# matthewdm0816/BridgeQA

Measured on AMD Instinct MI355X. Metric: train samples/s (40k-pt scene + 512^2 view, bs16), higher is better.
Workload: dtype bf16

## Files before the change

### bridgeqa_amd/csrc/gemm_mid.hip

```cpp
#include "gemm_common.h"

#ifndef BQ_MID_ABLATE
#define BQ_MID_ABLATE 0
#endif

namespace bq {

typedef __attribute__((address_space(3))) unsigned char lds_u8_t;
typedef unsigned u32x2_t __attribute__((ext_vector_type(2)));
typedef unsigned u32x4_t __attribute__((ext_vector_type(4)));

template <bool P_XC, bool Q_XC, int EPI, bool OUT_F32, int ST_AUX, bool SK = false>
__global__ __launch_bounds__(256, 2) void gemm128_kernel(const GemmArgs args) {
  static_assert(!OUT_F32 || (P_XC && Q_XC && EPI == EPI_NONE), "fp32 out = the weight-gradient form");
  static_assert(!Q_XC || OUT_F32, "a contraction-major Q = the weight-gradient form");
  static_assert(!SK || (!OUT_F32 && EPI != EPI_BIAS_GELU), "stream-K: bf16 out, one output");
  __shared__ __attribute__((aligned(16))) unsigned char smem[65536 + 4 * 2048 + (SK ? 16 : 0)];
  const int tid = threadIdx.x;
  const int lane = tid & 63;
  const int wave = __builtin_amdgcn_readfirstlane(tid >> 6);
  const int wr = wave >> 1, wc = wave & 1;
  const int nwg = args.total_tiles, G = (int)gridDim.x;

  const int row16 = lane & 15, q4 = lane >> 4, cp = lane & 7, lr = lane >> 3;
  const int kc_base = row16 * 128 + ((q4 ^ (row16 & 7)) << 4);
  const int xc_q = (lane & 15) >> 2;
  const int xcg = (xc_q >> 1) | ((q4 & 1) << 1), xc0 = (8 * q4 + xc_q) * 128 + 8 * (lane & 3);
  constexpr int PA0 = 0, PA1 = 16384, QB = 32768;
  const int uA0 = PA0 + wr * 8192, uA1 = PA1 + wr * 8192;
  const int bsub = wc * 2;

  struct Tile { int pi, i0, j0, nkt, kt0, t; };
  auto xcd_order = [](int v, int n) {
    const int q = n >> 3, r = n & 7, x = v & 7;
    return (x < r ? x * (q + 1) : r * (q + 1) + (x - r) * q) + (v >> 3);
  };
  auto decode_t = [&](int t) {
    int pi = 0;
    for (int k = 1; k < args.n; ++k)
      if (t >= args.p[k].tile0) pi = k;
    const GemmProblem &pr = args.p[pi];
    const int tl = t - pr.tile0;
    const int tiles_j = (pr.Nj + 127) >> 7;
    Tile tt;
    tt.pi = pi;
    tt.j0 = (tiles_j - 1 - tl / pr.tiles_i()) * 128;
    tt.i0 = (tl % pr.tiles_i()) * 256;
    tt.nkt = (pr.Kc + 63) >> 6;
    tt.kt0 = 0;
    tt.t = t;
    return tt;
  };
  auto decode = [&](int v) { return decode_t(xcd_order(v, nwg)); };
  const int nkt_full = SK ? (args.p[0].Kc + 63) >> 6 : 1;
  const int U = SK ? nwg * nkt_full : 0;
  auto bound = [&](int x) {
    int b = (int)((long)x * U / G);
    const int r = b % nkt_full;
    return r == 1 ? b - 1 : (r == nkt_full - 1 ? b + 1 : b);
  };
  auto seg = [&](int u, int ue) {
    const int t = u / nkt_full;
    Tile tt = decode_t(t);
    tt.kt0 = u - t * nkt_full;
    const int left = nkt_full - tt.kt0;
    tt.nkt = left < ue - u ? left : ue - u;
    return tt;
  };
  const int slot = SK ? xcd_order((int)blockIdx.x, G) : 0;
  int su = SK ? bound(slot) : 0;
  const int sue = SK ? bound(slot + 1) : 0;

  unsigned vP[2], vQ[2];
  unsigned stepP[2], dgP[2], ddP[2], ddQ[2], stepQ[2];
  int remP[2], remQ[2];
  int rsrcP_pi[2], rsrcQ_pi[2];
  const unsigned DEAD = 0x80000000u;
  const int ur0 = wave * 8 + lr;

  auto set_p = [&](int half, const Tile &tt, bool live) {
    const GemmProblem &pr = args.p[tt.pi];
    const int ldp = pr.ldp;
    unsigned v;
    if (!P_XC) v = (unsigned)(((tt.i0 + half * 64 + ur0) * ldp + (cp ^ (ur0 & 7)) * 8) * 2);
    else v = (unsigned)((ur0 * ldp + tt.i0 + half * 64 + (cp ^ (xg(ur0) << 1)) * 8) * 2);
    stepP[half] = P_XC ? (unsigned)(64 * ldp * 2) : 128u;
    if (SK) v += (unsigned)tt.kt0 * stepP[half];
    vP[half] = live ? v : DEAD;
    dgP[half] = P_XC ? 256u : (unsigned)(128 * ldp * 2);
    ddP[half] = (unsigned)(32 * ldp * 2);
    remP[half] = live ? tt.nkt : 0x40000000;
    rsrcP_pi[half] = tt.pi;
  };
  auto set_q = [&](int half, const Tile &tt, bool live) {
    const GemmProblem &pr = args.p[tt.pi];
    unsigned v;
    if (!Q_XC) {
      const int row0 = tt.j0 + half * 32 + ur0;
      const unsigned o0 = mapped_row(row0, pr.ldq, pr.q_rpb(), pr.q_bstride);
      v = (o0 + (unsigned)((cp ^ (ur0 & 7)) * 8)) * 2u;
      ddQ[half] = pr.q_rpb() ? (mapped_row(row0 + 64, pr.ldq, pr.q_rpb(), pr.q_bstride) - o0) * 2u : (unsigned)(64 * pr.ldq * 2);
    } else {
      const int c = cp ^ (xg(ur0) << 1);
      v = (unsigned)((ur0 * pr.ldq + tt.j0 + (c >> 2) * 64 + half * 32 + (c & 3) * 8) * 2);
      ddQ[half] = (unsigned)(32 * pr.ldq * 2);
    }
    stepQ[half] = Q_XC ? (unsigned)(64 * pr.ldq * 2) : 128u;
    if (SK) v += (unsigned)tt.kt0 * stepQ[half];
    vQ[half] = live ? v : DEAD;
    remQ[half] = live ? tt.nkt : 0x40000000;
    rsrcQ_pi[half] = tt.pi;
  };

  int v = blockIdx.x;
  Tile cur = SK ? seg(su, sue) : decode(v);
  bool has_next = SK ? (su + cur.nkt < sue) : (v + G < nwg);
  Tile nxt = has_next ? (SK ? seg(su + cur.nkt, sue) : decode(v + G)) : cur;

  auto dma_p = [&](int half) {
    const GemmProblem &pr = args.p[rsrcP_pi[half]];
    const auto rs = __builtin_amdgcn_make_buffer_rsrc((void *)pr.P, 0, pr.p_bytes, 0x00020000);
#pragma unroll
    for (int g = 0; g < 2; ++g)
#pragma unroll
      for (int d = 0; d < 2; ++d)
        if (BQ_MID_ABLATE != 2)
          __builtin_amdgcn_raw_ptr_buffer_load_lds(rs, (lds_void_t *)(smem + (half ? PA1 : PA0) + g * 8192 + (wave + 4 * d) * 1024),
                                                   16, vP[half] + (g * dgP[half] + d * ddP[half]), 0, 0, 0);
    vP[half] += stepP[half];
    if (--remP[half] == 0) set_p(half, nxt, has_next);
  };
  auto dma_q = [&](int half, unsigned par) {
    const GemmProblem &pr = args.p[rsrcQ_pi[half]];
    const auto rs = __builtin_amdgcn_make_buffer_rsrc((void *)pr.Q, 0, pr.q_bytes, 0x00020000);
#pragma unroll
    for (int d = 0; d < 2; ++d)
      if (BQ_MID_ABLATE != 2)
        __builtin_amdgcn_raw_ptr_buffer_load_lds(rs, (lds_void_t *)(smem + QB + (par & 1) * 16384 + half * 8192 + (wave + 4 * d) * 1024),
                                                 16, vQ[half] + d * ddQ[half], 0, 0, 0);
    vQ[half] += Q_XC ? stepQ[half] : 128u;
    if (--remQ[half] == 0) set_q(half, nxt, has_next);
  };

  set_q(0, cur, true); set_q(1, cur, true); set_p(0, cur, true); set_p(1, cur, true);
  unsigned gk = 0;
  dma_q(0, 0); dma_q(1, 0); dma_p(0); dma_q(0, 1); dma_p(1);

  f32x4 acc[8][4];
  bf16x8 fa[4][2], fb0[2][2], fb1[2][2];
#define BQ_MID_MFMA(AO, FB, BO)                                                                       \
  _Pragma("unroll") for (int kk = 0; kk < 2; ++kk) _Pragma("unroll") for (int a = 0; a < 4; ++a)      \
      _Pragma("unroll") for (int b = 0; b < 2; ++b) if (BQ_MID_ABLATE != 1 || (a == 0 && b == 0)) acc[AO + a][BO + b] =  \
          __builtin_amdgcn_mfma_f32_16x16x32_bf16(fa[a][kk], FB[b][kk], acc[AO + a][BO + b], 0, 0, 0);
#define BQ_MID_COMPUTE_BEGIN()                              \
  asm volatile("s_waitcnt lgkmcnt(0)" ::: "memory");        \
  __builtin_amdgcn_sched_barrier(0);                        \
  __builtin_amdgcn_s_setprio(1);
#define BQ_MID_COMPUTE_END()                                \
  __builtin_amdgcn_s_setprio(0);                            \
  __builtin_amdgcn_sched_barrier(0);
  constexpr int NPASS = (EPI == EPI_BIAS_GELU) ? 2 : 1;
  constexpr int NSTORE = OUT_F32 ? 36 : 16 * NPASS;
  bf16x8 ones;
  f32x4 qs[4];
  if (OUT_F32) {
#pragma unroll
    for (int e = 0; e < 8; ++e) ones[e] = (__bf16)1.0f;
  }
#define BQ_MID_QSUM(FB, BO)                                                                           \
  if (OUT_F32 && do_qsum) {                                                                           \
    _Pragma("unroll") for (int kk = 0; kk < 2; ++kk) _Pragma("unroll") for (int b = 0; b < 2; ++b)    \
        qs[BO + b] = __builtin_amdgcn_mfma_f32_16x16x32_bf16(ones, FB[b][kk], qs[BO + b], 0, 0, 0);   \
  }

  for (bool first = true;; first = false) {
    const GemmProblem &pr = args.p[cur.pi];
    const int Ni = pr.Ni, Nj = pr.Nj;
    const int iw = cur.i0 + wr * 128, jw = cur.j0 + wc * 64;
    const bool vA0 = iw < Ni, vA1 = iw + 64 < Ni, vB0 = jw < Nj, vB1 = jw + 32 < Nj;
#pragma unroll
    for (int a = 0; a < 8; ++a)
#pragma unroll
      for (int b = 0; b < 4; ++b) acc[a][b] = f32x4{0.f, 0.f, 0.f, 0.f};
    const bool do_qsum = OUT_F32 && pr.colsum != nullptr && cur.i0 == 0 && wr == 0;
    if (OUT_F32) {
#pragma unroll
      for (int b = 0; b < 4; ++b) qs[b] = f32x4{0.f, 0.f, 0.f, 0.f};
    }

    for (int kt = 0; kt < cur.nkt; ++kt, ++gk) {
      const unsigned char *qb = smem + QB + (gk & 1) * 16384;
      const bool after_stores = kt == 0 && !first;
      const bool last = kt == cur.nkt - 1;
      if (after_stores) wait_vmcnt<6 + NSTORE>(); else wait_vmcnt<6>();
      BQ_BARRIER();
#pragma unroll
      for (int a = 0; a < 4; ++a)
#pragma unroll
        for (int kk = 0; kk < 2; ++kk) fa[a][kk] = read_frag_cf_x<P_XC>(smem + uA0, a, kk, kc_base, xc0, xcg);
#pragma unroll
      for (int b = 0; b < 2; ++b)
#pragma unroll
        for (int kk = 0; kk < 2; ++kk) fb0[b][kk] = read_frag_cf_x<Q_XC>(qb, bsub + b, kk, kc_base, xc0, xcg);
      dma_q(1, gk + 1);
      BQ_MID_COMPUTE_BEGIN();
      if (vA0 && vB0) { BQ_MID_MFMA(0, fb0, 0) }
      if (vB0) { BQ_MID_QSUM(fb0, 0) }
      BQ_MID_COMPUTE_END();
      BQ_BARRIER();
#pragma unroll
      for (int b = 0; b < 2; ++b)
#pragma unroll
        for (int kk = 0; kk < 2; ++kk) fb1[b][kk] = read_frag_cf_x<Q_XC>(qb + 8192, bsub + b, kk, kc_base, xc0, xcg);
      dma_p(0);
      BQ_MID_COMPUTE_BEGIN();
      if (vA0 && vB1) { BQ_MID_MFMA(0, fb1, 2) }
      if (vB1) { BQ_MID_QSUM(fb1, 2) }
      BQ_MID_COMPUTE_END();
      if (after_stores) wait_vmcnt<6 + NSTORE>(); else wait_vmcnt<6>();
      BQ_BARRIER();
#pragma unroll
      for (int a = 0; a < 4; ++a)
#pragma unroll
        for (int kk = 0; kk < 2; ++kk) fa[a][kk] = read_frag_cf_x<P_XC>(smem + uA1, a, kk, kc_base, xc0, xcg);
      if (!last) dma_q(0, gk + 2);
      BQ_MID_COMPUTE_BEGIN();
      if (vA1 && vB1) { BQ_MID_MFMA(4, fb1, 2) }
      BQ_MID_COMPUTE_END();
      BQ_BARRIER();
      if (!last) dma_p(1);
      __builtin_amdgcn_sched_barrier(0);
      __builtin_amdgcn_s_setprio(1);
      if (vA1 && vB0) { BQ_MID_MFMA(4, fb0, 0) }
      BQ_MID_COMPUTE_END();
    }

    bool sk_partial = false;
    if (SK && cur.nkt != nkt_full) {
      unsigned *tick = (unsigned *)args.sk_ws + 2 * cur.t;
      float *slabs = (float *)((char *)args.sk_ws + SK_TICKET_BYTES);
      const int t0 = cur.t * nkt_full, t1 = t0 + nkt_full;
      int s_lo = slot, s_hi = slot;
      while (s_lo > 0 && bound(s_lo) > t0) --s_lo;
      while (s_hi + 1 < G && bound(s_hi + 1) < t1) ++s_hi;
      const int n_part = s_hi - s_lo + 1;
      const unsigned flag_lds = (unsigned)(size_t)((lds_u8_t *)smem) + 65536u + 4u * 2048u;
      if (wave == 0) {
        unsigned old = 0;
        if (lane == 0) old = __hip_atomic_fetch_add(tick, 1u, __ATOMIC_RELAXED, __HIP_MEMORY_SCOPE_AGENT);
        old = (unsigned)__builtin_amdgcn_readfirstlane((int)old);
        asm volatile("ds_write_b32 %0, %1\n\ts_waitcnt lgkmcnt(0)" ::"v"(flag_lds), "v"(old) : "memory");
      }
      BQ_BARRIER();
      unsigned arrived;
      asm volatile("ds_read_b32 %0, %1\n\ts_waitcnt lgkmcnt(0)" : "=v"(arrived) : "v"(flag_lds) : "memory");
      arrived = (unsigned)__builtin_amdgcn_readfirstlane((int)arrived);
      const auto rsW = __builtin_amdgcn_make_buffer_rsrc((void *)slabs, 0, (unsigned)(2 * G) * (unsigned)SK_SLAB_BYTES > 0x7fffffffu
                                                         ? 0x7fffffffu : (unsigned)(2 * G) * (unsigned)SK_SLAB_BYTES, 0x00020000);
      auto slab_off = [&](int sl) { return (unsigned)((2 * sl + (bound(sl) >= t0 ? 0 : 1))) * (unsigned)SK_SLAB_BYTES; };
      if (arrived != (unsigned)(n_part - 1)) {
        sk_partial = true;
        __builtin_amdgcn_sched_barrier(0);
        dma_q(0, gk + 1);
        dma_p(1);
        __builtin_amdgcn_sched_barrier(0);
        const unsigned base = slab_off(slot) + (unsigned)(wave * 32 * 1024 + lane * 16);
#pragma unroll
        for (int a = 0; a < 8; ++a)
#pragma unroll
          for (int b = 0; b < 4; ++b)
            __builtin_amdgcn_raw_buffer_store_b128(__builtin_bit_cast(u32x4_t, acc[a][b]), rsW, base + (unsigned)((a * 4 + b) * 1024), 0, 16);
        asm volatile("s_waitcnt vmcnt(0)" ::: "memory");
        BQ_BARRIER();
        if (wave == 0 && lane == 0) __hip_atomic_fetch_add(tick + 1, 1u, __ATOMIC_RELAXED, __HIP_MEMORY_SCOPE_AGENT);
      } else {
        if (wave == 0 && lane == 0) {
          for (int spin = 0; spin < (1 << 22) && __hip_atomic_load(tick + 1, __ATOMIC_RELAXED, __HIP_MEMORY_SCOPE_AGENT) != (unsigned)(n_part - 1); ++spin)
            __builtin_amdgcn_s_sleep(4);
          __hip_atomic_store(tick, 0u, __ATOMIC_RELAXED, __HIP_MEMORY_SCOPE_AGENT);
          __hip_atomic_store(tick + 1, 0u, __ATOMIC_RELAXED, __HIP_MEMORY_SCOPE_AGENT);
        }
        BQ_BARRIER();
        for (int sl = s_lo; sl <= s_hi; ++sl) {
          if (sl == slot) continue;
          const unsigned base = slab_off(sl) + (unsigned)(wave * 32 * 1024 + lane * 16);
#pragma unroll
          for (int a0 = 0; a0 < 8; a0 += 4) {
            u32x4_t part[16];
#pragma unroll
            for (int e = 0; e < 16; ++e)
              part[e] = __builtin_amdgcn_raw_buffer_load_b128(rsW, base + (unsigned)((a0 * 4 + e) * 1024), 0, 16);
            asm volatile("s_waitcnt vmcnt(0)" ::: "memory");
            __builtin_amdgcn_sched_barrier(0);
#pragma unroll
            for (int e = 0; e < 16; ++e) acc[a0 + (e >> 2)][e & 3] += __builtin_bit_cast(f32x4, part[e]);
          }
        }
      }
    }

    if (SK && sk_partial) {
    } else if (OUT_F32) {
      __builtin_amdgcn_sched_barrier(0);
      dma_q(0, gk + 1);
      dma_p(1);
      __builtin_amdgcn_sched_barrier(0);
      const int ldo = pr.ldo;
      const auto rsO = __builtin_amdgcn_make_buffer_rsrc(pr.out, 0, (unsigned)((long)Nj * ldo * 4), 0x00020000);
      const auto rsS = __builtin_amdgcn_make_buffer_rsrc((void *)pr.colsum, 0, pr.colsum == nullptr ? 0u : (unsigned)(Nj * 4), 0x00020000);
#pragma unroll
      for (int b = 0; b < 4; ++b) {
        const int j = jw + b * 16 + row16;
        __builtin_amdgcn_raw_buffer_store_b32(__float_as_uint(qs[b][0]), rsS, (do_qsum && q4 == 0) ? (unsigned)(j * 4) : DEAD, 0, 0);
      }
#pragma unroll
      for (int b = 0; b < 4; ++b) {
        const int j = jw + b * 16 + row16;
#pragma unroll
        for (int a = 0; a < 8; ++a) {
          const int i = iw + a * 16 + q4 * 4;
          const unsigned off = i < Ni ? (unsigned)((j * ldo + i) * 4) : DEAD;
          __builtin_amdgcn_raw_buffer_store_b128(__builtin_bit_cast(u32x4_t, acc[a][b]), rsO, off, 0, ST_AUX);
        }
      }
    } else {
      const int ldo = pr.ldo;
      const int orpb = pr.o_rpb(), obs = pr.o_bstride;
      const unsigned obytes = orpb ? (unsigned)((long)(Nj / orpb) * obs * 2) : (unsigned)((long)Nj * ldo * 2);
      const auto rsO = __builtin_amdgcn_make_buffer_rsrc(pr.out, 0, obytes, 0x00020000);
      const auto rsO2 = __builtin_amdgcn_make_buffer_rsrc(EPI == EPI_BIAS_GELU ? pr.out2 : pr.out, 0, obytes, 0x00020000);
      const auto rsX = __builtin_amdgcn_make_buffer_rsrc((void *)((EPI == EPI_DGELU || EPI == EPI_ADD) ? (const void *)pr.aux : pr.out), 0, obytes, 0x00020000);
      const int wj = row16 * 128 + (q4 & 1) * 8, wx = row16 & 7, wc2 = q4 >> 1;
      auto deferred_dmas = [&]() {
        __builtin_amdgcn_sched_barrier(0);
        dma_q(0, gk + 1);
        dma_p(1);
        __builtin_amdgcn_sched_barrier(0);
      };
      if (EPI == EPI_BIAS || EPI == EPI_BIAS_GELU) {
        float bias_r[8][4];
        const bool bb = pr.bias_bf16() != 0;
        const auto rsB = __builtin_amdgcn_make_buffer_rsrc((void *)pr.bias, 0, pr.bias == nullptr ? 0 : Ni * (bb ? 2 : 4), 0x00020000);
        const unsigned bo = (unsigned)(iw + q4 * 4);
        if (bb) {
          uint2 raw[8];
#pragma unroll
          for (int a = 0; a < 8; ++a) raw[a] = __builtin_bit_cast(uint2, __builtin_amdgcn_raw_buffer_load_b64(rsB, (bo + a * 16) * 2, 0, 0));
#pragma unroll
          for (int a = 0; a < 8; ++a) {
            bias_r[a][0] = __uint_as_float(raw[a].x << 16); bias_r[a][1] = __uint_as_float(raw[a].x & 0xffff0000u);
            bias_r[a][2] = __uint_as_float(raw[a].y << 16); bias_r[a][3] = __uint_as_float(raw[a].y & 0xffff0000u);
          }
        } else {
#pragma unroll
          for (int a = 0; a < 8; ++a) {
            const float4 t4 = __builtin_bit_cast(float4, __builtin_amdgcn_raw_buffer_load_b128(rsB, (bo + a * 16) * 4, 0, 0));
            bias_r[a][0] = t4.x; bias_r[a][1] = t4.y; bias_r[a][2] = t4.z; bias_r[a][3] = t4.w;
          }
        }
        deferred_dmas();
#pragma unroll
        for (int a = 0; a < 8; ++a)
#pragma unroll
          for (int b = 0; b < 4; ++b)
#pragma unroll
            for (int r = 0; r < 4; ++r) acc[a][b][r] += bias_r[a][r];
      } else if (EPI == EPI_DGELU || EPI == EPI_ADD) {
        uint2 yA[8], yB[8];
        auto fetch = [&](int b, uint2(&dst)[8]) {
          const unsigned off = (mapped_row(jw + b * 16 + row16, ldo, orpb, obs) + (unsigned)(iw + q4 * 4)) * 2u;
#pragma unroll
          for (int a = 0; a < 8; ++a)
            dst[a] = __builtin_bit_cast(uint2, __builtin_amdgcn_raw_buffer_load_b64(rsX, off + a * 32, 0, 0));
          __builtin_amdgcn_sched_barrier(0);
        };
        auto fold = [&](auto b_tag, const uint2(&src)[8]) {
          constexpr int b = decltype(b_tag)::value;
#pragma unroll
          for (int a = 0; a < 8; ++a) {
            const uint2 yb = src[a];
            const float y0 = __uint_as_float(yb.x << 16), y1 = __uint_as_float(yb.x & 0xffff0000u);
            const float y2 = __uint_as_float(yb.y << 16), y3 = __uint_as_float(yb.y & 0xffff0000u);
            if (EPI == EPI_DGELU) {
              acc[a][b][0] *= dgelu_f(y0); acc[a][b][1] *= dgelu_f(y1); acc[a][b][2] *= dgelu_f(y2); acc[a][b][3] *= dgelu_f(y3);
              __builtin_amdgcn_sched_barrier(0);
            } else {
              acc[a][b][0] += y0; acc[a][b][1] += y1; acc[a][b][2] += y2; acc[a][b][3] += y3;
            }
          }
          __builtin_amdgcn_sched_barrier(0);
        };
        typedef std::integral_constant<int, 0> B0; typedef std::integral_constant<int, 1> B1;
        typedef std::integral_constant<int, 2> B2; typedef std::integral_constant<int, 3> B3;
        fetch(0, yA); fetch(1, yB);
        fold(B0{}, yA);
        fetch(2, yA);
        fold(B1{}, yB);
        fetch(3, yB);
        deferred_dmas();
        fold(B2{}, yA);
        fold(B3{}, yB);
      } else {
        deferred_dmas();
      }
      const unsigned ep_lds = (unsigned)(size_t)((lds_u8_t *)smem) + 65536u + (unsigned)(wave * 2048);
      unsigned jrow[4][2];
#pragma unroll
      for (int b = 0; b < 4; ++b)
#pragma unroll
        for (int t2 = 0; t2 < 2; ++t2) jrow[b][t2] = mapped_row(jw + b * 16 + t2 * 8 + lr, ldo, orpb, obs);
#pragma unroll
      for (int b = 0; b < 4; ++b) {
#pragma unroll
        for (int pass = 0; pass < NPASS; ++pass) {
#pragma unroll
          for (int half = 0; half < 2; ++half) {
#pragma unroll
            for (int a4 = 0; a4 < 4; ++a4) {
              const int a = half * 4 + a4;
              float vv[4];
#pragma unroll
              for (int r = 0; r < 4; ++r) vv[r] = (float)(__bf16)acc[a][b][r];
              if (EPI == EPI_BIAS_GELU && pass == 1) {
#pragma unroll
                for (int r = 0; r < 4; ++r) vv[r] = gelu_f(vv[r]);
              }
              const u32x2_t pk = {pack_bf16x2(vv[0], vv[1]), pack_bf16x2(vv[2], vv[3])};
              asm volatile("ds_write_b64 %0, %1" ::"v"(ep_lds + (unsigned)(wj + (((a4 * 2 + wc2) ^ wx) << 4))), "v"(pk) : "memory");
            }
            asm volatile("s_waitcnt lgkmcnt(0)" ::: "memory");
            __builtin_amdgcn_sched_barrier(0);
            u32x4_t d[2];
#pragma unroll
            for (int t2 = 0; t2 < 2; ++t2) {
              const int jr = t2 * 8 + lr;
              asm volatile("ds_read_b128 %0, %1" : "=v"(d[t2]) : "v"(ep_lds + (unsigned)(jr * 128 + ((cp ^ (jr & 7)) << 4))) : "memory");
            }
            asm volatile("s_waitcnt lgkmcnt(0)" : "+v"(d[0]), "+v"(d[1])::"memory");
            __builtin_amdgcn_sched_barrier(0);
#pragma unroll
            for (int t2 = 0; t2 < 2; ++t2) {
              const int i_st = iw + half * 64 + cp * 8;
              const unsigned off = i_st < Ni ? (jrow[b][t2] + (unsigned)i_st) * 2u : DEAD;
              __builtin_amdgcn_raw_buffer_store_b128(d[t2], pass == 1 ? rsO2 : rsO, off, 0, ST_AUX);
            }
          }
        }
      }
    }

    if (SK) {
      su += cur.nkt;
      if (su >= sue) break;
      cur = nxt;
      has_next = su + cur.nkt < sue;
      if (has_next) nxt = seg(su + cur.nkt, sue);
    } else {
      v += G;
      if (v >= nwg) break;
      cur = nxt;
      has_next = v + G < nwg;
      if (has_next) nxt = decode(v + G);
    }
  }
  asm volatile("s_waitcnt vmcnt(0)" ::: "memory");
}

struct SkWorkspace { int device; hipStream_t stream; void *ptr; long bytes; };
static SkWorkspace g_sk_ws[16];
static int g_sk_n = 0;

void *gemm_sk_workspace(hipStream_t st, long *bytes) {
  int dev = 0;
  if (hipGetDevice(&dev) != hipSuccess) return nullptr;
  for (int i = 0; i < g_sk_n; ++i)
    if (g_sk_ws[i].device == dev && g_sk_ws[i].stream == st) {
      *bytes = g_sk_ws[i].bytes;
      return g_sk_ws[i].ptr;
    }
  return nullptr;
}

static int g_sk_mode = 0;
int gemm_sk_mode() {
  static int env_off = -1;
  if (env_off < 0) {
    const char *e = getenv("BQ_GEMM_STREAMK");
    env_off = (e != nullptr && e[0] == '0') ? 1 : 0;
  }
  return env_off ? 0 : g_sk_mode;
}

int launch_gemm_mid(const GemmArgs &ga_in, bool p_xc, bool q_xc, bool out_f32, int epi, bool background, hipStream_t stream) {
  const int slots = 2 * device_cus();
  for (int k = 0; k < ga_in.n; ++k)
    if (ga_in.p[k].Kc < 128) return -1;
  GemmArgs ga = ga_in;
  ga.sk_ws = nullptr;
  if ((gemm_sk_mode() & 1) && !background && ga.n == 1 && !p_xc && !q_xc && !out_f32 && (epi == EPI_NONE || epi == EPI_BIAS || epi == EPI_ADD)) {
    long ws_bytes = 0;
    void *ws = gemm_sk_workspace(stream, &ws_bytes);
    if (streamk_fits((ga.p[0].Kc + 63) >> 6, ga.total_tiles, slots, SK_SLAB_BYTES, ws, ws_bytes)) {
      ga.sk_ws = ws;
      with_int<EPI_NONE, EPI_BIAS, EPI_ADD>(epi, [&](auto E) {
        static_assert(gemm_form(128, false, false, false, decltype(E)::value, FORM_STREAMK), "not a stream-K form");
        hipLaunchKernelGGL((gemm128_kernel<false, false, decltype(E)::value, false, 16, true>), dim3(slots), dim3(256), 0, stream, ga);
      });
      return 0;
    }
  }
  for (int k = 0; k < ga.n; ++k)
    if (!out_f32 && ga.p[k].colsum != nullptr) return -1;
  const int use = background ? (slots + 1) / 2 : slots;
  const dim3 grid(ga.total_tiles < use ? ga.total_tiles : use), block(256);
  int rc = -1;
  with_gemm_form(p_xc, q_xc, out_f32, epi, [&](auto PX, auto QX, auto F32, auto E) {
    if constexpr (gemm_form(128, decltype(PX)::value, decltype(QX)::value, decltype(F32)::value, decltype(E)::value)) {
      hipLaunchKernelGGL((gemm128_kernel<decltype(PX)::value, decltype(QX)::value, decltype(E)::value, decltype(F32)::value, 16>),
                         grid, block, 0, stream, ga);
      rc = 0;
    }
  });
  return rc;
}

}

extern "C" int bq_gemm_streamk_mode(int mode) {
  const int old = bq::g_sk_mode;
  if (mode >= 0) bq::g_sk_mode = mode & 3;
  return old;
}

extern "C" long bq_gemm_workspace_bytes(void) {
  return bq::SK_TICKET_BYTES + 2L * 2L * bq::device_cus() * bq::SK_SLAB_BYTES;
}

extern "C" int bq_gemm_set_workspace(void *ws, long bytes, void *stream) {
  using namespace bq;
  int dev = 0;
  BQ_REQUIRE(hipGetDevice(&dev) == hipSuccess, BQ_EINVAL, "bq_gemm_set_workspace: no device");
  BQ_REQUIRE(ws == nullptr || bytes >= bq_gemm_workspace_bytes(), BQ_EINVAL, "bq_gemm_set_workspace: %ld bytes < %ld", bytes,
             bq_gemm_workspace_bytes());
  for (int i = 0; i < g_sk_n; ++i)
    if (g_sk_ws[i].device == dev && g_sk_ws[i].stream == (hipStream_t)stream) {
      g_sk_ws[i].ptr = ws;
      g_sk_ws[i].bytes = bytes;
      return 0;
    }
  BQ_REQUIRE(g_sk_n < 16, BQ_ELIMIT, "bq_gemm_set_workspace: more than 16 (device, stream) pairs");
  g_sk_ws[g_sk_n++] = SkWorkspace{dev, (hipStream_t)stream, ws, bytes};
  return 0;
}
```

Measured before the change: 514.5.

## Precompute next-tile DMA cursors and cache buffer descriptors in scalar registers

Next-tile address setup moves out of the DMA lambdas into one set_next call made once per tile. Its results, including the base pointer and size for each buffer resource, are held in scalar registers pinned with inline asm. The DMA helpers then build buffer descriptors from the cached words instead of reloading the problem struct from kernarg memory on every issue. They simply swap in the precomputed cursor when a tile finishes. The deferred DMAs in the epilogue no longer roll over, and the q0 cursor is advanced after the tile loop step instead. This should cut scalar loads and branchy setup from the inner loop, at the cost of more SGPR pressure and riskier rollover ordering logic.

```diff
diff --git a/bridgeqa_amd/csrc/gemm_mid.hip b/bridgeqa_amd/csrc/gemm_mid.hip
--- a/bridgeqa_amd/csrc/gemm_mid.hip
+++ b/bridgeqa_amd/csrc/gemm_mid.hip
@@ -72,78 +72,115 @@
   const int sue = SK ? bound(slot + 1) : 0;
 
   unsigned vP[2], vQ[2];
-  unsigned stepP[2], dgP[2], ddP[2], ddQ[2], stepQ[2];
+  unsigned ddQ[2];
+  unsigned ddP[2], stepQ[2];
   int remP[2], remQ[2];
-  int rsrcP_pi[2], rsrcQ_pi[2];
+  unsigned bufP[2][3], bufQ[2][3];
   const unsigned DEAD = 0x80000000u;
   const int ur0 = wave * 8 + lr;
 
-  auto set_p = [&](int half, const Tile &tt, bool live) {
+#define BQ_MID_STEP_P(dd) (P_XC ? 2u * (dd) : 128u)
+#define BQ_MID_DG_P(dd) (P_XC ? 256u : 4u * (dd))
+  struct Next {
+    unsigned vP[2], vQ[2], ddQ[2];
+    unsigned ddP, stepQ, bufP[3], bufQ[3];
+    int nkt;
+  } nx;
+#if defined(__HIP_DEVICE_COMPILE__)
+#define BQ_MID_PIN(x) asm volatile("" : "+s"(x))
+#else
+#define BQ_MID_PIN(x) (void)(x)
+#endif
+  auto set_next = [&](const Tile &tt, bool live) {
     const GemmProblem &pr = args.p[tt.pi];
-    const int ldp = pr.ldp;
-    unsigned v;
-    if (!P_XC) v = (unsigned)(((tt.i0 + half * 64 + ur0) * ldp + (cp ^ (ur0 & 7)) * 8) * 2);
-    else v = (unsigned)((ur0 * ldp + tt.i0 + half * 64 + (cp ^ (xg(ur0) << 1)) * 8) * 2);
-    stepP[half] = P_XC ? (unsigned)(64 * ldp * 2) : 128u;
-    if (SK) v += (unsigned)tt.kt0 * stepP[half];
-    vP[half] = live ? v : DEAD;
-    dgP[half] = P_XC ? 256u : (unsigned)(128 * ldp * 2);
-    ddP[half] = (unsigned)(32 * ldp * 2);
-    remP[half] = live ? tt.nkt : 0x40000000;
-    rsrcP_pi[half] = tt.pi;
-  };
-  auto set_q = [&](int half, const Tile &tt, bool live) {
-    const GemmProblem &pr = args.p[tt.pi];
-    unsigned v;
-    if (!Q_XC) {
-      const int row0 = tt.j0 + half * 32 + ur0;
-      const unsigned o0 = mapped_row(row0, pr.ldq, pr.q_rpb(), pr.q_bstride);
-      v = (o0 + (unsigned)((cp ^ (ur0 & 7)) * 8)) * 2u;
-      ddQ[half] = pr.q_rpb() ? (mapped_row(row0 + 64, pr.ldq, pr.q_rpb(), pr.q_bstride) - o0) * 2u : (unsigned)(64 * pr.ldq * 2);
-    } else {
-      const int c = cp ^ (xg(ur0) << 1);
-      v = (unsigned)((ur0 * pr.ldq + tt.j0 + (c >> 2) * 64 + half * 32 + (c & 3) * 8) * 2);
-      ddQ[half] = (unsigned)(32 * pr.ldq * 2);
-    }
-    stepQ[half] = Q_XC ? (unsigned)(64 * pr.ldq * 2) : 128u;
-    if (SK) v += (unsigned)tt.kt0 * stepQ[half];
-    vQ[half] = live ? v : DEAD;
-    remQ[half] = live ? tt.nkt : 0x40000000;
-    rsrcQ_pi[half] = tt.pi;
-  };
-
+    const int ldp = pr.ldp, ldq = pr.ldq;
+    nx.stepQ = Q_XC ? (unsigned)(64 * ldq * 2) : 128u;
+    nx.ddP = (unsigned)(32 * ldp * 2);
+    nx.nkt = live ? tt.nkt : 0x40000000;
+    const unsigned long pa = (unsigned long)pr.P, qa = (unsigned long)pr.Q;
+    nx.bufP[0] = (unsigned)pa; nx.bufP[1] = (unsigned)(pa >> 32); nx.bufP[2] = pr.p_bytes;
+    nx.bufQ[0] = (unsigned)qa; nx.bufQ[1] = (unsigned)(qa >> 32); nx.bufQ[2] = pr.q_bytes;
+    BQ_MID_PIN(nx.stepQ); BQ_MID_PIN(nx.ddP); BQ_MID_PIN(nx.nkt);
+#pragma unroll
+    for (int e = 0; e < 3; ++e) { BQ_MID_PIN(nx.bufP[e]); BQ_MID_PIN(nx.bufQ[e]); }
+#pragma unroll
+    for (int half = 0; half < 2; ++half) {
+      unsigned v;
+      if (!P_XC) v = (unsigned)(((tt.i0 + half * 64 + ur0) * ldp + (cp ^ (ur0 & 7)) * 8) * 2);
+      else v = (unsigned)((ur0 * ldp + tt.i0 + half * 64 + (cp ^ (xg(ur0) << 1)) * 8) * 2);
+      if (SK) v += (unsigned)tt.kt0 * BQ_MID_STEP_P(nx.ddP);
+      nx.vP[half] = live ? v : DEAD;
+      if (!Q_XC) {
+        const int row0 = tt.j0 + half * 32 + ur0;
+        const unsigned o0 = mapped_row(row0, ldq, pr.q_rpb(), pr.q_bstride);
+        v = (o0 + (unsigned)((cp ^ (ur0 & 7)) * 8)) * 2u;
+        nx.ddQ[half] = pr.q_rpb() ? (mapped_row(row0 + 64, ldq, pr.q_rpb(), pr.q_bstride) - o0) * 2u : (unsigned)(64 * ldq * 2);
+      } else {
+        const int c = cp ^ (xg(ur0) << 1);
+        v = (unsigned)((ur0 * ldq + tt.j0 + (c >> 2) * 64 + half * 32 + (c & 3) * 8) * 2);
+        nx.ddQ[half] = (unsigned)(32 * ldq * 2);
+      }
+      if (SK) v += (unsigned)tt.kt0 * nx.stepQ;
+      nx.vQ[half] = live ? v : DEAD;
+    }
+  };
+  auto take_p = [&](int half) {
+    vP[half] = nx.vP[half];
+    ddP[half] = nx.ddP;
+    remP[half] = nx.nkt;
+#pragma unroll
+    for (int e = 0; e < 3; ++e) bufP[half][e] = nx.bufP[e];
+  };
+  auto take_q = [&](int half) {
+    vQ[half] = nx.vQ[half];
+    ddQ[half] = nx.ddQ[half];
+    stepQ[half] = nx.stepQ;
+    remQ[half] = nx.nkt;
+#pragma unroll
+    for (int e = 0; e < 3; ++e) bufQ[half][e] = nx.bufQ[e];
+  };
+#define BQ_MID_CURSOR_RSRC(b) __builtin_amdgcn_make_buffer_rsrc((void *)(((unsigned long)(b)[1] << 32) | (b)[0]), 0, (b)[2], 0x00020000)
+
+  unsigned gk = 0;
   int v = blockIdx.x;
   Tile cur = SK ? seg(su, sue) : decode(v);
   bool has_next = SK ? (su + cur.nkt < sue) : (v + G < nwg);
   Tile nxt = has_next ? (SK ? seg(su + cur.nkt, sue) : decode(v + G)) : cur;
 
-  auto dma_p = [&](int half) {
-    const GemmProblem &pr = args.p[rsrcP_pi[half]];
-    const auto rs = __builtin_amdgcn_make_buffer_rsrc((void *)pr.P, 0, pr.p_bytes, 0x00020000);
+  auto dma_p = [&](int half, bool roll = true) {
+    const auto rs = BQ_MID_CURSOR_RSRC(bufP[half]);
 #pragma unroll
     for (int g = 0; g < 2; ++g)
 #pragma unroll
       for (int d = 0; d < 2; ++d)
         if (BQ_MID_ABLATE != 2)
           __builtin_amdgcn_raw_ptr_buffer_load_lds(rs, (lds_void_t *)(smem + (half ? PA1 : PA0) + g * 8192 + (wave + 4 * d) * 1024),
-                                                   16, vP[half] + (g * dgP[half] + d * ddP[half]), 0, 0, 0);
-    vP[half] += stepP[half];
-    if (--remP[half] == 0) set_p(half, nxt, has_next);
-  };
-  auto dma_q = [&](int half, unsigned par) {
-    const GemmProblem &pr = args.p[rsrcQ_pi[half]];
-    const auto rs = __builtin_amdgcn_make_buffer_rsrc((void *)pr.Q, 0, pr.q_bytes, 0x00020000);
+                                                   16, vP[half] + (g * BQ_MID_DG_P(ddP[half]) + d * ddP[half]), 0, 0, 0);
+    vP[half] += BQ_MID_STEP_P(ddP[half]);
+    --remP[half];
+    if (roll && remP[half] == 0) take_p(half);
+  };
+  auto dma_q = [&](int half, unsigned par, bool roll = true) {
+    const auto rs = BQ_MID_CURSOR_RSRC(bufQ[half]);
 #pragma unroll
     for (int d = 0; d < 2; ++d)
       if (BQ_MID_ABLATE != 2)
         __builtin_amdgcn_raw_ptr_buffer_load_lds(rs, (lds_void_t *)(smem + QB + (par & 1) * 16384 + half * 8192 + (wave + 4 * d) * 1024),
                                                  16, vQ[half] + d * ddQ[half], 0, 0, 0);
     vQ[half] += Q_XC ? stepQ[half] : 128u;
-    if (--remQ[half] == 0) set_q(half, nxt, has_next);
-  };
-
-  set_q(0, cur, true); set_q(1, cur, true); set_p(0, cur, true); set_p(1, cur, true);
-  unsigned gk = 0;
+    --remQ[half];
+    if (roll && remQ[half] == 0) take_q(half);
+  };
+  auto deferred_dmas = [&]() {
+    __builtin_amdgcn_sched_barrier(0);
+    dma_q(0, gk + 1, false);
+    dma_p(1, false);
+    __builtin_amdgcn_sched_barrier(0);
+  };
+
+  set_next(cur, true);
+  take_q(0); take_q(1); take_p(0); take_p(1);
+  set_next(nxt, has_next);
   dma_q(0, 0); dma_q(1, 0); dma_p(0); dma_q(0, 1); dma_p(1);
 
   f32x4 acc[8][4];
@@ -260,10 +297,7 @@
       auto slab_off = [&](int sl) { return (unsigned)((2 * sl + (bound(sl) >= t0 ? 0 : 1))) * (unsigned)SK_SLAB_BYTES; };
       if (arrived != (unsigned)(n_part - 1)) {
         sk_partial = true;
-        __builtin_amdgcn_sched_barrier(0);
-        dma_q(0, gk + 1);
-        dma_p(1);
-        __builtin_amdgcn_sched_barrier(0);
+        deferred_dmas();
         const unsigned base = slab_off(slot) + (unsigned)(wave * 32 * 1024 + lane * 16);
 #pragma unroll
         for (int a = 0; a < 8; ++a)
@@ -301,10 +335,7 @@
 
     if (SK && sk_partial) {
     } else if (OUT_F32) {
-      __builtin_amdgcn_sched_barrier(0);
-      dma_q(0, gk + 1);
-      dma_p(1);
-      __builtin_amdgcn_sched_barrier(0);
+      deferred_dmas();
       const int ldo = pr.ldo;
       const auto rsO = __builtin_amdgcn_make_buffer_rsrc(pr.out, 0, (unsigned)((long)Nj * ldo * 4), 0x00020000);
       const auto rsS = __builtin_amdgcn_make_buffer_rsrc((void *)pr.colsum, 0, pr.colsum == nullptr ? 0u : (unsigned)(Nj * 4), 0x00020000);
@@ -331,12 +362,6 @@
       const auto rsO2 = __builtin_amdgcn_make_buffer_rsrc(EPI == EPI_BIAS_GELU ? pr.out2 : pr.out, 0, obytes, 0x00020000);
       const auto rsX = __builtin_amdgcn_make_buffer_rsrc((void *)((EPI == EPI_DGELU || EPI == EPI_ADD) ? (const void *)pr.aux : pr.out), 0, obytes, 0x00020000);
       const int wj = row16 * 128 + (q4 & 1) * 8, wx = row16 & 7, wc2 = q4 >> 1;
-      auto deferred_dmas = [&]() {
-        __builtin_amdgcn_sched_barrier(0);
-        dma_q(0, gk + 1);
-        dma_p(1);
-        __builtin_amdgcn_sched_barrier(0);
-      };
       if (EPI == EPI_BIAS || EPI == EPI_BIAS_GELU) {
         float bias_r[8][4];
         const bool bb = pr.bias_bf16() != 0;
@@ -462,6 +487,8 @@
       has_next = v + G < nwg;
       if (has_next) nxt = decode(v + G);
     }
+    set_next(nxt, has_next);
+    if (remQ[0] == 0) take_q(0);
   }
   asm volatile("s_waitcnt vmcnt(0)" ::: "memory");
 }
```

Result: no change. 511.6 (-0.6%).
